# bldeng/AA-ADMM

Measured on AMD Instinct MI355X. Metric: ADMM iters/sec + time-to-eps (primal+dual residual), higher is better.
Workload: dtype f64

## Files before the change

aa-admm_amd/csrc/elastic.cpp:

```cpp
#include "elastic.hpp"

#include <algorithm>
#include <chrono>
#include <cmath>
#include <cstdio>
#include <cstdlib>
#include <cstring>
#include <memory>
#include <numeric>
#include <set>

#include "dense_gpu.hpp"
#include "spd_direct.hpp"

namespace aa {

ElasticSolver::~ElasticSolver() {
    drop_graph();
    if (ev_fork_) (void)hipEventDestroy(ev_fork_);
    if (ev_join_) (void)hipEventDestroy(ev_join_);
    if (side_) (void)hipStreamDestroy(side_);
    for (auto& kv : kstats_)
        for (auto e : kv.second.ev) (void)hipEventDestroy(e);
}
// ... 440 lines not shown
            double v = 0;
            while (k2 < r.size() && r[k2].first == r[k].first) v += r[k2++].second;
            out.push_back({r[k].first, v});
            k = k2;
        }
        rows[q] = std::move(out);
    }
    CsrMatrix A;
    A.n = nf_;
    A.ptr.assign(nf_ + 1, 0);
    for (int q = 0; q < nf_; ++q) A.ptr[q + 1] = A.ptr[q] + (int)rows[q].size();
    A.col.resize(A.ptr[nf_]);
    A.val.resize(A.ptr[nf_]);
#pragma omp parallel for schedule(static)
    for (int q = 0; q < nf_; ++q)
        for (size_t k = 0; k < rows[q].size(); ++k) { A.col[A.ptr[q] + k] = rows[q][k].first; A.val[A.ptr[q] + k] = rows[q][k].second; }
    std::vector<std::vector<std::pair<int, double>>>().swap(rows);
    stamp("assembly of A_s");
    SupernodalFactor F;
    try {
        auto pf = make_part_factor(P > 1 ? comm_ : nullptr, rank_, s());
        F = factor_on_device(A, tree, s(), pf.get());
    } catch (const Error&) {
        throw;
    } catch (const std::runtime_error& e) {
        throw Error(ERR_NUMERIC, e.what());
    }
    pipe_z_ = st_.variant == AA_VARIANT_Z && st_.acceleration_type == 1;
    if (const char* e = std::getenv("AA_Z_PIPELINE")) pipe_z_ = pipe_z_ && e[0] != '0';
    conc_ = pipe_z_ && !comm_;
    if (const char* e = std::getenv("AA_CONCURRENT")) conc_ = conc_ && e[0] != '0';
    win_u_ = conc_;
    if (const char* e = std::getenv("AA_Z_WINDOW")) win_u_ = win_u_ && e[0] != '0';
    stamp("factor");
    solver_.default_branches = (P == 1 && st_.variant == AA_VARIANT_Z) ? 2 : 1;
    solver_.build(F, s(), P > 1 ? &tree.part : nullptr, rank_, top_beg_, comm_, pipe_z_ ? 2 : 1,
                  st_.variant == AA_VARIANT_Z && st_.acceleration_type == 1);
    stamp("solver build + upload");

    std::vector<HostGroup> owned;
    nbg_ = 0;
    long long zmax = 0;
    if (P > 1) {
        std::vector<int> qpart(n, -1);
        for (int r = 0; r < P; ++r) for (int q = tree.part_beg[r]; q < tree.part_end[r]; ++q) qpart[q] = r;
        std::vector<long long> zr(P, 0);
        std::vector<int> br(P, 0);
        long long rr = 0;
        for (auto& hg : hgroups_) {
            const int cnt = (int)(hg.idx.size() / hg.nv);
            std::vector<int> c(P, 0);
            HostGroup lg;
            lg.kind = hg.kind; lg.material = hg.material; lg.nv = hg.nv; lg.ncol = hg.ncol; lg.lame = hg.lame;
            for (int t = 0; t < cnt; ++t) {
                int o = -1;
                for (int a = 0; a < hg.nv && o < 0; ++a) o = qpart[node2int_[hg.idx[(size_t)t * hg.nv + a]]];
                if (o < 0) o = (int)(rr++ % P);
                ++c[o];
                if (o != rank_) continue;
                lg.append_element(hg, (size_t)t);
            }
            for (int r = 0; r < P; ++r) { br[r] += blocks_for(c[r]); zr[r] += 3LL * hg.ncol * c[r]; }
            owned.push_back(std::move(lg));
        }
        for (int r = 0; r < P; ++r) { nbg_ = std::max(nbg_, br[r]); zmax = std::max(zmax, zr[r]); }
    }
// ... 222 lines not shown
    if (!pins_dirty_) return;
    std::vector<double> p(3 * (size_t)np_);
    int q = 0;
    for (auto& kv : pins_) { for (int j = 0; j < 3; ++j) p[3 * q + j] = kv.second[j]; ++q; }
    if (np_) {
        const size_t off = 3 * (size_t)nf_;
        AA_HIP(hipMemcpyAsync(xfull_.p + off, p.data(), p.size() * 8, hipMemcpyHostToDevice, s()));
        AA_HIP(hipMemcpyAsync(xlast_.p + off, p.data(), p.size() * 8, hipMemcpyHostToDevice, s()));
        AA_HIP(hipMemcpyAsync(cxfull_.p + off, p.data(), p.size() * 8, hipMemcpyHostToDevice, s()));
        AA_HIP(hipStreamSynchronize(s()));
    }
    pins_dirty_ = false;
}

void ElasticSolver::ev_begin(const char* name) {
    if (!instrument_) return;
    hipEvent_t e;
    AA_HIP(hipEventCreate(&e));
    AA_HIP(hipEventRecord(e, s()));
    kstats_[name].ev.push_back(e);
}
void ElasticSolver::ev_end(const char* name) { ev_begin(name); }

void ElasticSolver::local_z_all(const double* xfull, const double* u, double* z, double* y, int mode, bool red) {
    int off = 0;
    const bool timed = mode == LZ_NORMAL && red;
    if (timed) ev_begin("local_z");
    for (auto& g : groups_) {
        launch_local_z(g.d, xfull, u, z, y, nf_, st_.variant, mode, ctrl_.p, red ? pa_ : nullptr, off, s(),
                       use_queue_ ? &lq_ : nullptr, g.var, mesh_table(g.d));
        off += blocks_for(g.d.count);
    }
    if (timed) ev_end("local_z");
}

void ElasticSolver::local_z_on(const double* xfull, const double* u, double* z, int mode, hipStream_t st, Ctrl* c,
                               const LocalQueue* q) {
    for (auto& g : groups_)
        launch_local_z(g.d, xfull, u, z, nullptr, nf_, st_.variant, mode, c, nullptr, 0, st, use_queue_ ? q : nullptr,
                       g.var, mesh_table(g.d));
}

void ElasticSolver::prologue() {
    upload_pins();
    const bool accel = st_.acceleration_type == 1;
    Ctrl c;
    std::memset(&c, 0, sizeof(c));
    c.prev_prim = 1e20;
    c.cap = hist_cap_;
    c.aa_m = accel ? st_.anderson_m : 0;
    c.aa_active = accel ? 1 : 0;
    c.hist_clock = hist_clock_.p;
    c.eps_rel = st_.eps_rel;
    AA_HIP(hipMemcpyAsync(ctrl_.p, &c, sizeof(Ctrl), hipMemcpyHostToDevice, s()));
    launch_stamp(ctrl_.p, s());
    for (auto& w : winds_)
        launch_wind(w->dtris.p, w->dord.p, w->dlvl.p, w->nlvl, xs_.p, vs_.p, w->dir[0], w->dir[1], w->dir[2],
                    st_.timestep_s, s());
    launch_predict(n_, nf_, xs_.p, vs_.p, mass_.p, st_.timestep_s, st_.gravity, xbar_.p, Mxbar_.p, xfull_.p, s());
    if (comm_ && rank_ != 0 && top_beg_ < nf_)
        AA_HIP(hipMemsetAsync(Mxbar_.p + 3 * (size_t)top_beg_, 0, 3 * sizeof(double) * (size_t)(nf_ - top_beg_), s()));
    for (auto& g : groups_) launch_init_z(g.d, xfull_.p, z_.p, s());
    double* u0 = u_at(-1);
    if (Z_) AA_HIP(hipMemsetAsync(u0, 0, sizeof(double) * (size_t)Z_, s()));
    const long long nx = 3LL * nf_;
    if (st_.variant == AA_VARIANT_UX) {
        local_z_all(xfull_.p, u_.p, z_.p, y_.p, LZ_INIT, false);
        launch_rhs(nf_, dt_ptr_.p, nullptr, nullptr, y_.p, Mxbar_.p, pdt2_, b_.p, nullptr, 0, s());
        solver_.solve(b_.p, xfull_.p, nullptr, 0, s());
        {
            int off = 0;
            for (auto& g : groups_) {
                launch_resid_update_u(g.d, xfull_.p, xlast_.p, z_.p, u_.p, nf_, ctrl_.p, pa_, pb_, off, s());
// ... 24 lines not shown
    reduce_partials();
    launch_check_restore_ux(c, ga_, nbg_, accel, u_.p, xfull_.p, accel ? aa_cur_.p : nullptr, du_.p, dx_.p,
                            Z_, nx, s());
    if (accel) {
        local_z_all(xfull_.p, u_.p, z_.p, y_.p, LZ_REDO, true);
        reduce_partials();
    }
    ev_begin("rhs");
    launch_rhs(nf_, dt_ptr_.p, nullptr, nullptr, y_.p, Mxbar_.p, pdt2_, b_.p, c, 0, s(), xfull_.p, xlast_.p,
               ga_, nbg_);
    ev_end("rhs");
    ev_begin("solve");
    solver_.solve(b_.p, xfull_.p, c, 0, s());
    ev_end("solve");
    ev_begin("resid");
    {
        int off = 0;
        for (auto& g : groups_) {
            launch_resid_update_u(g.d, xfull_.p, xlast_.p, z_.p, u_.p, nf_, c, pa_, pb_, off, s());
            off += blocks_for(g.d.count);
        }
    }
    ev_end("resid");
    reduce_partials();
    if (accel) {
        const int m = st_.anderson_m;
        Seg2 G{u_.p, Z_, xfull_.p, nx};
        Seg2 cp{du_.p, Z_, dx_.p, nx};
        ev_begin("aa");
        launch_aa_reduce(G, aa_cur_.p, Z_, aa_dF_.p, aa_dG_.p, c, aa_red_.p, aa_blocks_, cp, m, s(), ga_, gb_, nbg_,
                         hist_prim_.p, hist_comb_.p, hist_rej_.p);
        reduce_aa();
        launch_aa_solve(c, aag_, aa_blocks_, m, s());
        launch_aa_mix(G, aa_cur_.p, Z_, aa_dF_.p, aa_dG_.p, c, G, m, s());
        ev_end("aa");
    } else {
        launch_control(CTL_COMB_UX, c, ga_, gb_, nbg_, accel, hist_prim_.p, hist_comb_.p, hist_rej_.p, s());
    }
}

void ElasticSolver::enqueue_iteration_z(bool accel, int it) {
    const long long nx = 3LL * nf_;
    Ctrl* c = ctrl_.p;
    const bool pipe = accel && pipe_z_;
    double *duc = du_at(it), *dzc = dz_at(it), *dxc = dx_at(it);
    double *dup = du_at(it - 1), *dzp = dz_at(it - 1), *dxp = dx_at(it - 1);
    const bool side = pipe && it > 0 && conc_;
    auto side_pass = [&](hipStream_t st) {
        comb_finish_z(CTL_COMB_ZP, st, ctrl_c_.p, red_c_.p, red_c_.p + nbg_, &lq2_, dup, dzp);
    };
    double* u = u_at(it);
    const double* ui = win_u_ ? dup : u_.p;
    ev_begin("grad");
    for (auto& g : groups_) launch_u_and_y(g.d, xfull_.p, z_.p, u, u, y_.p, nf_, accel ? 1 : 0, 0, c, s(), g.var);
    ev_end("grad");
    ev_begin("rhs");
    launch_rhs(nf_, dt_ptr_.p, nullptr, nullptr, y_.p, Mxbar_.p, pdt2_, b_.p, c, 0, s());
    ev_end("rhs");
    if (pipe && it > 0) {
        ev_begin("solve");
        solver_.solve2(b_.p, xfull_.p, b2_.p, cxfull_.p, c, 0, s());
        ev_end("solve");
        if (side) {
            launch_ctrl_fork(c, ctrl_c_.p, s());
        } else {
            ev_begin("comb");
            comb_finish_z(CTL_COMB_ZP, s(), c, pa_, pb_, &lq_, dup, dzp);
// ... 30 lines not shown
    if (accel) {
        const int m = st_.anderson_m;
        auto copy_defaults = [&]() {
            ev_begin("copy");
            launch_copy(dxc, xfull_.p, nx, c, 0, s());
            if (!win_u_) launch_copy(duc, u_.p, Z_, c, 0, s());
            ev_end("copy");
        };
        if (instrument_) copy_defaults();
        ev_begin("local_z");
        local_z_all(xfull_.p, u, dzc, y_.p, LZ_NORMAL, false);
        ev_end("local_z");
        if (side && instrument_) {
            ev_begin("comb");
            side_pass(s());
            ev_end("comb");
            join_wait_ = false;
        }
        Seg2 G{dzc, Z_, nullptr, 0};
        Seg2 out{z_.p, Z_, nullptr, 0};
        Seg2 none{nullptr, 0, nullptr, 0};
        ev_begin("aa");
        launch_aa_reduce(G, z_.p, Z_, aa_dF_.p, aa_dG_.p, c, aa_red_.p, aa_blocks_, none, m, s());
        reduce_aa();
        if (side && !instrument_) {
            AA_HIP(hipEventRecord(ev_fork_, s()));
            AA_HIP(hipStreamWaitEvent(side_, ev_fork_, 0));
            side_pass(side_);
            AA_HIP(hipEventRecord(ev_join_, side_));
            join_wait_ = true;
        }
        if (!instrument_) copy_defaults();
        launch_aa_solve(c, aag_, aa_blocks_, m, s());
        launch_aa_mix(G, z_.p, Z_, aa_dF_.p, aa_dG_.p, c, out, m, s());
        ev_end("aa");
        if (pipe) {
            ev_begin("rhs");
            launch_rhs(nf_, dt_ptr_.p, nullptr, nullptr, y_.p, Mxbar_.p, pdt2_, b2_.p, c, 0, s());
            ev_end("rhs");
            if (side) {
                join_dx_ = dxp;
                join_side();
            }
            return;
        }
        ev_begin("comb");
        launch_rhs(nf_, dt_ptr_.p, nullptr, nullptr, y_.p, Mxbar_.p, pdt2_, b_.p, c, 0, s());
        solver_.solve(b_.p, cxfull_.p, c, 0, s());
        comb_finish_z(CTL_COMB_Z, s(), c, pa_, pb_, &lq_, duc, dzc);
        ev_end("comb");
        return;
    }
    launch_copy(lastz_.p, z_.p, Z_, c, 0, s());
    ev_begin("local_z");
    local_z_all(xfull_.p, u, z_.p, nullptr, LZ_NORMAL, false);
    ev_end("local_z");
    prim_all(xfull_.p, z_.p, lastz_.p, 0);
    reduce_partials();
    launch_control(CTL_COMB_Z, c, ga_, gb_, nbg_, accel, hist_prim_.p, hist_comb_.p, hist_rej_.p, s());
}

void ElasticSolver::comb_finish_z(int op, hipStream_t st, Ctrl* c, double* pa, double* pb, const LocalQueue* q,
                                  const double* du, const double* dz) {
    local_z_on(cxfull_.p, du, cz_.p, LZ_NORMAL, st, c, q);
    int off = 0;
    for (auto& g : groups_) {
        launch_prim_z(g.d, cxfull_.p, cz_.p, dz, nf_, 0, c, pa, pb, off, st);
        off += blocks_for(g.d.count);
    }
    if (st == s()) {
        reduce_partials();
        launch_control(op, c, ga_, gb_, nbg_, 1, hist_prim_.p, hist_comb_.p, hist_rej_.p, st);
    } else {
        launch_control(op, c, pa, pb, nbg_, 1, hist_prim_.p, hist_comb_.p, hist_rej_.p, st);
    }
}

void ElasticSolver::join_side() {
    if (join_wait_) AA_HIP(hipStreamWaitEvent(s(), ev_join_, 0));
    launch_ctrl_join(ctrl_.p, ctrl_c_.p, xfull_.p, join_dx_, 3LL * nf_, s());
}

void ElasticSolver::enqueue_comb_tail_z(int iters) {
    ev_begin("comb");
    solver_.solve(b2_.p, cxfull_.p, ctrl_.p, 0, s());
    comb_finish_z(CTL_COMB_Z, s(), ctrl_.p, pa_, pb_, &lq_, du_at(iters - 1), dz_at(iters - 1));
    ev_end("comb");
}

void ElasticSolver::enqueue_iterations(int iters, bool accel) {
    static const int eager_sync = [] { const char* e = std::getenv("AA_EAGER_SYNC"); return e ? std::atoi(e) : 0; }();
    hipStreamCaptureStatus cst = hipStreamCaptureStatusNone;
    if (eager_sync > 0) AA_HIP(hipStreamIsCapturing(s(), &cst));
    for (int it = 0; it < iters; ++it) {
        if (st_.variant == AA_VARIANT_UX) enqueue_iteration_ux(accel);
        else enqueue_iteration_z(accel, it);
        if (eager_sync > 0 && cst == hipStreamCaptureStatusNone && (it + 1) % eager_sync == 0)
            AA_HIP(hipStreamSynchronize(s()));
    }
    if (st_.variant != AA_VARIANT_UX && accel && pipe_z_ && iters > 0) enqueue_comb_tail_z(iters);
// ... 179 lines not shown
```

aa-admm_amd/csrc/elastic.hpp:

```cpp
#pragma once
#include <array>
#include <map>
#include <memory>
#include <string>
#include <vector>

#include "../../include/aa_admm.h"
#include "comm.hpp"
#include "common.hpp"
#include "direct_solve.hpp"
#include "elastic_kernels.hpp"
#include "mesh_obstacle.hpp"

namespace aa {

struct Context {
    int device = 0;
    hipStream_t stream = nullptr;
};

struct MeshObsBuffers {
    DevBuf<BvhNode> nodes;
    DevBuf<BvhTri> tris;
    DevBuf<double> pn;
// ... 120 lines not shown
    int red_blocks_ = 0, aa_blocks_ = 0, hist_cap_ = 0;
    Comm* comm_ = nullptr;
    int rank_ = 0, own_beg_ = 0, own_end_ = 0, top_beg_ = 0;
    void reduce_partials();
    void reduce_aa();
    void gather_state(DevBuf<double>& v);
    std::vector<double> h_prim_, h_comb_;
    std::vector<int> h_rej_;
    int nrec_ = 0;
    aa_runtime rt_{};
    std::vector<std::pair<std::string, double>> setup_phases_;
    bool pins_dirty_ = true;

    hipGraph_t graph_ = nullptr;
    hipGraphExec_t gexec_ = nullptr;
    bool use_graph_ = true;
    bool pipe_z_ = false;
    void drop_graph();
    bool conc_ = false;
    bool join_wait_ = false;
    double* join_dx_ = nullptr;
    void join_side();
    hipStream_t side_ = nullptr;
    hipEvent_t ev_fork_ = nullptr, ev_join_ = nullptr;
    DevBuf<Ctrl> ctrl_c_;
    DevBuf<int> lzq2_;
    LocalQueue lq2_;
    DevBuf<double> red_c_, du2_, dz2_, dx2_;
    double* du_at(int it) { return conc_ && (it & 1) ? du2_.p : du_.p; }
    double* dz_at(int it) { return conc_ && (it & 1) ? dz2_.p : dz_.p; }
    double* dx_at(int it) { return conc_ && (it & 1) ? dx2_.p : dx_.p; }
    bool win_u_ = false;
    double* u_at(int it) { return win_u_ ? du_at(it) : u_.p; }

    bool instrument_ = false;
    struct KStat { std::vector<hipEvent_t> ev; double bytes = 0; double total_ms = 0; int launches = 0; };
    std::map<std::string, KStat> kstats_;
    void ev_begin(const char* name);
    void ev_end(const char* name);

    void upload_pins();
    void prologue();
    void enqueue_iteration_ux(bool accel);
    void enqueue_iteration_z(bool accel, int it);
    void comb_finish_z(int op, hipStream_t st, Ctrl* c, double* pa, double* pb, const LocalQueue* q,
                       const double* du, const double* dz);
    void enqueue_comb_tail_z(int iters);
    void enqueue_iterations(int iters, bool accel);
    void epilogue_enqueue(bool accel);
    void fetch_results();
    int nb_elems() const { return red_blocks_; }
    void local_z_all(const double* xfull, const double* u, double* z, double* y, int mode, bool red);
    void local_z_on(const double* xfull, const double* u, double* z, int mode, hipStream_t st, Ctrl* c,
                    const LocalQueue* q);
};

}
```

aa-admm_amd/csrc/elastic_kernels.hip:

```cpp
#include <algorithm>
#include <cstdlib>

#include "common.hpp"
#include "device_lbfgs.hpp"
#include "device_prox.hpp"
#include "elastic_kernels.hpp"

namespace aa {

namespace {

__device__ __forceinline__ double wave_sum(double v) {
#pragma unroll
    for (int o = 32; o > 0; o >>= 1) v += __shfl_down(v, o, 64);
    return v;
}

__device__ __forceinline__ double block_sum(double v, double* sm) {
    v = wave_sum(v);
    const int lane = threadIdx.x & 63, wid = threadIdx.x >> 6;
    if (lane == 0) sm[wid] = v;
    __syncthreads();
    double r = 0;
    if (threadIdx.x == 0)
// ... 124 lines not shown
    double gk[NC * NV];
#pragma unroll
    for (int a = 0; a < NV; ++a) pos[a] = g.spos[(size_t)a * g.count + e];
#pragma unroll
    for (int k = 0; k < NC * NV; ++k) gk[k] = g.G[(size_t)k * g.count + e];
#pragma unroll
    for (int a = 0; a < NV; ++a) {
        if (pos[a] < 0) continue;
        double f0 = 0, f1 = 0, f2 = 0;
#pragma unroll
        for (int c = 0; c < NC; ++c) {
            const double gc = gk[c * NV + a];
            f0 += gc * yc[3 * c]; f1 += gc * yc[3 * c + 1]; f2 += gc * yc[3 * c + 2];
        }
        double* o = y + 3 * (size_t)pos[a];
        o[0] = f0; o[1] = f1; o[2] = f2;
    }
}

template <int D>
__device__ __forceinline__ void load_u(const GroupDev& g, int e, const double* __restrict__ u, double* uu) {
    if (u) {
#pragma unroll
        for (int i = 0; i < D; ++i) uu[i] = u[g.zoff + (size_t)i * g.count + e];
    } else {
#pragma unroll
        for (int i = 0; i < D; ++i) uu[i] = 0.0;
    }
}

template <class... V>
constexpr bool kVar = sizeof...(V) != 0;
__device__ __forceinline__ const GroupVar& var_of(const GroupVar& v) { return v; }
template <bool VAR>
struct LaneMat {};
template <>
struct LaneMat<true> {
    double mu = 0, lambda = 0, k = 0;
};

template <int NV, int HYPER, class... V>
__global__ __launch_bounds__(kBlock) void k_local_z(GroupDev g, const double* __restrict__ xfull,
                                                    const double* __restrict__ u, double* __restrict__ z,
                                                    double* __restrict__ y, int nf, int variant, int mode, Ctrl* ctrl,
                                                    double* red, int red_off, V... gvp) {
    constexpr bool VAR = kVar<V...>;
    if (mode != LZ_INIT && gated(ctrl, mode == LZ_REDO)) return;
    __shared__ double sm[kBlock / 64];
    constexpr int NC = ncol_of(NV), D = 3 * NC;
    const int e = blockIdx.x * blockDim.x + threadIdx.x;
    double part = 0;
    if (e < g.count) {
        double F[D], Cp[D], uu[D], vin[D], zz[D];
        gather_F<NV>(g, e, xfull, nf, F, Cp);
        const double w = g.w[e];
        load_u<D>(g, e, u, uu);
#pragma unroll
        for (int i = 0; i < D; ++i) vin[i] = F[i] + uu[i] / w;
        if constexpr (NV == 1) {
            if (variant == 1) dev::collision_candidate(F, uu, w, vin);
            if constexpr (VAR) dev::collision_prox(vin, g.obs, zz, gvp...);
            else dev::collision_prox(vin, g.obs, zz);
        } else if constexpr (NV == 3) {
            if constexpr (VAR) dev::tri_prox(vin, zz, variant, var_of(gvp...).lmin[e], var_of(gvp...).lmax[e]);
            else dev::tri_prox(vin, zz, variant, g.lmin, g.lmax);
        } else if constexpr (HYPER == 0) {
// ... 122 lines not shown
                    }
                }
            }
        }
        bool fin = false;
        if constexpr (VAR) fin = active && L.iterate(g.mat, M.mu, M.lambda, M.k, vol, v, x, &fail);
        else fin = active && L.iterate(g.mat, g.mu, g.lambda, g.k, vol, v, x, &fail);
        if (fin) {
            active = false;
            pending = true;
            if (stats) atomicAdd(&hist[min(L.k_it, 100)], 1u);
        }
    }
    if (stats) {
        if (lane == 0) {
            atomicAdd(stats + 101, (unsigned long long)trips);
            atomicAdd(stats + 102, (unsigned long long)refills);
            atomicAdd(stats + 103, 1ull);
        }
        __syncthreads();
        for (int i = threadIdx.x; i < 101; i += blockDim.x)
            if (hist[i]) atomicAdd(stats + i, (unsigned long long)hist[i]);
    }
    if (fail && ctrl) ctrl->fail = 1;
    queue_reset_last(queue);
}

template <int NV, bool SLOTS = true, class... V>
__global__ __launch_bounds__(kBlock) void k_local_z_hqf(GroupDev g, const double* __restrict__ xfull,
                                                        const double* __restrict__ u, double* __restrict__ z,
                                                        double* __restrict__ y, int nf, int mode, Ctrl* ctrl,
                                                        int* __restrict__ queue, int refill,
                                                        unsigned long long* __restrict__ stats, V... gvp) {
    constexpr bool VAR = kVar<V...>;
    static_assert(NV == 4, "the fused refill is for tets");
    if (mode != LZ_INIT && gated(ctrl, mode == LZ_REDO)) return;
    unsigned trips = 0, refills = 0;
    __shared__ unsigned hist[101];
    if (stats) {
        for (int i = threadIdx.x; i < 101; i += blockDim.x) hist[i] = 0;
        __syncthreads();
    }
    constexpr int NC = ncol_of(NV), D = 3 * NC;
    const int lane = threadIdx.x & 63;
    dev::HyperLbfgs L;
    [[maybe_unused]] LaneMat<VAR> M;
    double v[D], x[D];
    double vol = 0;
    int e = 0, fail = 0;
    bool active = false, pending = false, exhausted = false;
    const size_t n = g.count;
    for (;;) {
        const bool need = !active && !exhausted;
        const unsigned long long mask = __ballot(need);
        if (!__any(active || need)) break;
        ++trips;
        if (mask && (__popcll(mask) >= refill || !__any(active))) {
            ++refills;
            const int leader = __ffsll((long long)mask) - 1;
            const int rank = __popcll(mask & ((1ull << lane) - 1ull));
            int b = 0;
            if (lane == leader) b = queue_claim(queue, __popcll(mask));
            int so[NV];
            double go[NC * NV], uo[D], wo = 1.0;
            if (SLOTS && y) {
#pragma unroll
                for (int a = 0; a < NV; ++a) so[a] = g.spos[a * n + e];
#pragma unroll
                for (int k = 0; k < NC * NV; ++k) go[k] = g.G[k * n + e];
                load_u<D>(g, e, u, uo);
                wo = g.w[e];
            }
            b = __shfl(b, leader, 64);
            const int my = b + rank;
            const int en = min(my, g.count - 1);
            int id[NV];
#pragma unroll
            for (int a = 0; a < NV; ++a) id[a] = g.idx[a * n + en];
            if (pending) {
#pragma unroll
                for (int i = 0; i < D; ++i) z[g.zoff + (size_t)i * n + e] = x[i];
                if (SLOTS && y) {
                    double Cp[D];
#pragma unroll
                    for (int i = 0; i < D; ++i) Cp[i] = 0;
                    write_slots_pre<NV>(so, go, wo, x, Cp, uo, y);
                }
                pending = false;
            }
            double xp[3 * NV], gn[NC * NV], un[D];
#pragma unroll
            for (int a = 0; a < NV; ++a) {
                xp[3 * a] = xfull[3 * (size_t)id[a]];
                xp[3 * a + 1] = xfull[3 * (size_t)id[a] + 1];
                xp[3 * a + 2] = xfull[3 * (size_t)id[a] + 2];
            }
#pragma unroll
            for (int k = 0; k < NC * NV; ++k) gn[k] = g.G[k * n + en];
            load_u<D>(g, en, u, un);
            const double wn = g.w[en], voln = g.vol[en];
            [[maybe_unused]] double mun = 0, lamn = 0, kn = 0;
            if constexpr (VAR) {
                const GroupVar& gv = var_of(gvp...);
                mun = gv.mu[en]; lamn = gv.lambda[en]; kn = gv.k[en];
            }
            if (need) {
                if (my >= g.count) {
                    exhausted = true;
                } else {
                    e = my;
                    double F[D];
#pragma unroll
                    for (int i = 0; i < D; ++i) F[i] = 0;
#pragma unroll
                    for (int a = 0; a < NV; ++a)
#pragma unroll
                        for (int c = 0; c < NC; ++c) {
                            const double gc = gn[c * NV + a];
                            F[3 * c + 0] += gc * xp[3 * a]; F[3 * c + 1] += gc * xp[3 * a + 1];
                            F[3 * c + 2] += gc * xp[3 * a + 2];
                        }
#pragma unroll
                    for (int i = 0; i < D; ++i) {
                        v[i] = F[i] + un[i] / wn;
                        x[i] = v[i];
                    }
                    vol = voln;
                    bool ok;
                    if constexpr (VAR) {
                        M.mu = mun; M.lambda = lamn; M.k = kn;
                        ok = L.start(g.mat, M.mu, M.lambda, M.k, vol, v, x);
                    } else {
                        ok = L.start(g.mat, g.mu, g.lambda, g.k, vol, v, x);
                    }
                    if (ok) {
                        pending = true;
                        if (stats) atomicAdd(&hist[0], 1u);
                    } else {
                        active = true;
                    }
                }
            }
        }
        bool fin = false;
        if constexpr (VAR) fin = active && L.iterate(g.mat, M.mu, M.lambda, M.k, vol, v, x, &fail);
        else fin = active && L.iterate(g.mat, g.mu, g.lambda, g.k, vol, v, x, &fail);
        if (fin) {
            active = false;
            pending = true;
            if (stats) atomicAdd(&hist[min(L.k_it, 100)], 1u);
        }
    }
    if (stats) {
        if (lane == 0) {
            atomicAdd(stats + 101, (unsigned long long)trips);
            atomicAdd(stats + 102, (unsigned long long)refills);
            atomicAdd(stats + 103, 1ull);
        }
// ... 231 lines not shown
}

template <int NV>
__global__ __launch_bounds__(kBlock) void k_prim_z(GroupDev g, const double* __restrict__ xfull,
                                                   const double* __restrict__ z, const double* __restrict__ zref,
                                                   int nf, int redo, Ctrl* ctrl, double* red_a, double* red_b,
                                                   int red_off) {
    if (gated(ctrl, redo)) return;
    __shared__ double sm[kBlock / 64];
    constexpr int NC = ncol_of(NV), D = 3 * NC;
    const int e = blockIdx.x * blockDim.x + threadIdx.x;
    double pa = 0, pb = 0;
    if (e < g.count) {
        double F[D];
        gather_P<NV>(g, e, xfull, F);
        const double w = g.w[e];
        double zi[D], zr[D];
#pragma unroll
        for (int i = 0; i < D; ++i) zi[i] = z[g.zoff + (size_t)i * g.count + e];
        if (zref) {
#pragma unroll
            for (int i = 0; i < D; ++i) zr[i] = zref[g.zoff + (size_t)i * g.count + e];
        }
#pragma unroll
        for (int i = 0; i < D; ++i) {
            const double r = w * (F[i] - zi[i]);
            pa += r * r;
            if (zref) { const double d = w * (zi[i] - zr[i]); pb += d * d; }
        }
    }
    const double sa = block_sum(pa, sm);
    const double sb = block_sum(pb, sm);
    if (threadIdx.x == 0) { red_a[red_off + blockIdx.x] = sa; if (red_b) red_b[red_off + blockIdx.x] = sb; }
}

template <int NV>
__global__ __launch_bounds__(kBlock) void k_init_z(GroupDev g, const double* __restrict__ xfull, double* __restrict__ z) {
    constexpr int NC = ncol_of(NV), D = 3 * NC;
    const int e = blockIdx.x * blockDim.x + threadIdx.x;
    if (e >= g.count) return;
    double F[D];
    gather_P<NV>(g, e, xfull, F);
#pragma unroll
    for (int i = 0; i < D; ++i) z[g.zoff + (size_t)i * g.count + e] = F[i];
}

__global__ __launch_bounds__(kBlock) void k_rhs(int nf, const int* __restrict__ ptr, const int* __restrict__ row,
                                                const double* __restrict__ val, const double* __restrict__ y,
                                                const double* __restrict__ Mxbar, double pdt2, double* __restrict__ b,
                                                Ctrl* ctrl, int gate_reject, const double* __restrict__ xsrc,
                                                double* __restrict__ xlast, const double* __restrict__ red_final,
                                                int nb_final) {
    if (gated(ctrl, gate_reject)) return;
    if (red_final && blockIdx.x == 0) {
        __shared__ double sm[kBlock / 64];
        const double a = block_sum_all(red_final, nb_final, sm);
        if (threadIdx.x == 0) {
            if (ctrl->reject) ctrl->prim = sqrt(a);
            ctrl->prev_prim = ctrl->prim;
        }
    }
    const int i = blockIdx.x * blockDim.x + threadIdx.x;
    if (i >= nf) return;
    if (xlast) {
        xlast[3 * (size_t)i] = xsrc[3 * (size_t)i];
        xlast[3 * (size_t)i + 1] = xsrc[3 * (size_t)i + 1];
// ... 825 lines not shown
        } else if (var) {
            const int rf = queue->refill_lanes;
            if (!queue->fused || g.pinned)
                hipLaunchKernelGGL((k_local_z_hq<4, GroupVar>), grid, dim3(kBlock), 0, s, g, xfull, u, z, y, nf, mode, ctrl,
                                   queue->counter, rf, queue->stats, var);
            else if (y)
                hipLaunchKernelGGL((k_local_z_hqf<4, true, GroupVar>), grid, dim3(kBlock), 0, s, g, xfull, u, z, y, nf, mode,
                                   ctrl, queue->counter, rf, queue->stats, var);
            else
                hipLaunchKernelGGL((k_local_z_hqf<4, false, GroupVar>), grid, dim3(kBlock), 0, s, g, xfull, u, z, y, nf,
                                   mode, ctrl, queue->counter, rf, queue->stats, var);
        } else if (!queue->fused || g.pinned)
            hipLaunchKernelGGL((k_local_z_hq<4>), grid, dim3(kBlock), 0, s, g, xfull, u, z, y, nf, mode, ctrl,
                               queue->counter, refill, queue->stats);
        else if (y)
            hipLaunchKernelGGL((k_local_z_hqf<4, true>), grid, dim3(kBlock), 0, s, g, xfull, u, z, y, nf, mode,
                               ctrl, queue->counter, refill, queue->stats);
        else
            hipLaunchKernelGGL((k_local_z_hqf<4, false>), grid, dim3(kBlock), 0, s, g, xfull, u, z, y, nf, mode,
                               ctrl, queue->counter, refill, queue->stats);
        AA_CHECK_LAUNCH();
        return;
    }
    if (g.kind == 2 && meshes) hipLaunchKernelGGL((k_local_z<1, 0, const MeshObsDev*>), dim3(nb), dim3(kBlock), 0, s, g, xfull, u, z, y, nf, variant, mode, ctrl, red, red_off, meshes);
    else if (g.kind == 2) hipLaunchKernelGGL((k_local_z<1, 0>), dim3(nb), dim3(kBlock), 0, s, g, xfull, u, z, y, nf, variant, mode, ctrl, red, red_off);
    else if (g.kind == 1 && var) hipLaunchKernelGGL((k_local_z<3, 0, GroupVar>), dim3(nb), dim3(kBlock), 0, s, g, xfull, u, z, y, nf, variant, mode, ctrl, red, red_off, var);
    else if (g.kind == 1) hipLaunchKernelGGL((k_local_z<3, 0>), dim3(nb), dim3(kBlock), 0, s, g, xfull, u, z, y, nf, variant, mode, ctrl, red, red_off);
    else if (g.mat == 0) hipLaunchKernelGGL((k_local_z<4, 0>), dim3(nb), dim3(kBlock), 0, s, g, xfull, u, z, y, nf, variant, mode, ctrl, red, red_off);
    else if (var) hipLaunchKernelGGL((k_local_z<4, 1, GroupVar>), dim3(nb), dim3(kBlock), 0, s, g, xfull, u, z, y, nf, variant, mode, ctrl, red, red_off, var);
    else hipLaunchKernelGGL((k_local_z<4, 1>), dim3(nb), dim3(kBlock), 0, s, g, xfull, u, z, y, nf, variant, mode, ctrl, red, red_off);
    AA_CHECK_LAUNCH();
}

void launch_resid_update_u(const GroupDev& g, const double* xfull, const double* xlast, const double* z, double* u,
                           int nf, Ctrl* ctrl, double* red_a, double* red_b, int red_off, hipStream_t s) {
    if (g.count == 0) return;
    const int nb = blocks_for(g.count);
    if (g.kind == 2) hipLaunchKernelGGL(k_resid_u<1>, dim3(nb), dim3(kBlock), 0, s, g, xfull, xlast, z, u, nf, ctrl, red_a, red_b, red_off);
    else if (g.kind == 1) hipLaunchKernelGGL(k_resid_u<3>, dim3(nb), dim3(kBlock), 0, s, g, xfull, xlast, z, u, nf, ctrl, red_a, red_b, red_off);
    else hipLaunchKernelGGL(k_resid_u<4>, dim3(nb), dim3(kBlock), 0, s, g, xfull, xlast, z, u, nf, ctrl, red_a, red_b, red_off);
    AA_CHECK_LAUNCH();
}

void launch_u_and_y(const GroupDev& g, const double* xfull, const double* z, const double* uin, double* u, double* y,
                    int nf, int mode, int redo, Ctrl* ctrl, hipStream_t s, const GroupVar& var) {
    if (g.count == 0) return;
    const int nb = blocks_for(g.count);
    if (g.kind == 2) hipLaunchKernelGGL((k_u_and_y<1, 0>), dim3(nb), dim3(kBlock), 0, s, g, xfull, z, uin, u, y, nf, mode, redo, ctrl);
    else if (g.kind == 1) hipLaunchKernelGGL((k_u_and_y<3, 0>), dim3(nb), dim3(kBlock), 0, s, g, xfull, z, uin, u, y, nf, mode, redo, ctrl);
    else if (g.mat == 0 && var) hipLaunchKernelGGL((k_u_and_y<4, 0, GroupVar>), dim3(nb), dim3(kBlock), 0, s, g, xfull, z, uin, u, y, nf, mode, redo, ctrl, var);
    else if (g.mat == 0) hipLaunchKernelGGL((k_u_and_y<4, 0>), dim3(nb), dim3(kBlock), 0, s, g, xfull, z, uin, u, y, nf, mode, redo, ctrl);
    else if (var) hipLaunchKernelGGL((k_u_and_y<4, 1, GroupVar>), dim3(nb), dim3(kBlock), 0, s, g, xfull, z, uin, u, y, nf, mode, redo, ctrl, var);
    else hipLaunchKernelGGL((k_u_and_y<4, 1>), dim3(nb), dim3(kBlock), 0, s, g, xfull, z, uin, u, y, nf, mode, redo, ctrl);
    AA_CHECK_LAUNCH();
}

void launch_prim_z(const GroupDev& g, const double* xfull, const double* z, const double* zref, int nf, int redo,
                   Ctrl* ctrl, double* red_a, double* red_b, int red_off, hipStream_t s) {
    if (g.count == 0) return;
    const int nb = blocks_for(g.count);
    if (g.kind == 2) hipLaunchKernelGGL(k_prim_z<1>, dim3(nb), dim3(kBlock), 0, s, g, xfull, z, zref, nf, redo, ctrl, red_a, red_b, red_off);
    else if (g.kind == 1) hipLaunchKernelGGL(k_prim_z<3>, dim3(nb), dim3(kBlock), 0, s, g, xfull, z, zref, nf, redo, ctrl, red_a, red_b, red_off);
    else hipLaunchKernelGGL(k_prim_z<4>, dim3(nb), dim3(kBlock), 0, s, g, xfull, z, zref, nf, redo, ctrl, red_a, red_b, red_off);
    AA_CHECK_LAUNCH();
}

// ... 163 lines not shown
static bool aa_cols() {
    static const bool on = !(std::getenv("AA_AA_COLS") && std::getenv("AA_AA_COLS")[0] == '0');
    return on;
}

void launch_aa_reduce(Seg2 G, const double* cur, long long eff, double* dF, double* dG, Ctrl* ctrl, double* red,
                      int nblocks, Seg2 copy_to, int m, hipStream_t s, const double* comb_a, const double* comb_b,
                      int comb_nb, double* hist_prim, double* hist_comb, int* hist_rej, AAMask mask) {
#define AA_RED_ARGS G, cur, eff, dF, dG, ctrl, red, copy_to, comb_a, comb_b, comb_nb, hist_prim, hist_comb, hist_rej, mask
    switch (mm_bucket(m)) {
        case 8: hipLaunchKernelGGL(k_aa_reduce<8>, dim3(nblocks), dim3(kBlock), 0, s, AA_RED_ARGS); break;
        case 12: hipLaunchKernelGGL(k_aa_reduce<12>, dim3(nblocks), dim3(kBlock), 0, s, AA_RED_ARGS); break;
        case 16: hipLaunchKernelGGL(k_aa_reduce<16>, dim3(nblocks), dim3(kBlock), 0, s, AA_RED_ARGS); break;
        default:
            if (aa_cols()) hipLaunchKernelGGL(k_aa_reduce_cols<32>, dim3(nblocks), dim3(kBlock), 0, s, AA_RED_ARGS);
            else hipLaunchKernelGGL(k_aa_reduce<32>, dim3(nblocks), dim3(kBlock), 0, s, AA_RED_ARGS);
            break;
    }
#undef AA_RED_ARGS
    AA_CHECK_LAUNCH();
}

void launch_aa_solve(Ctrl* ctrl, const double* red, int nblocks, int m, hipStream_t s) {
    switch (mm_bucket(m)) {
        case 8: hipLaunchKernelGGL(k_aa_solve<8>, dim3(1), dim3(kSolveBlock), 0, s, ctrl, red, nblocks); break;
        case 12: hipLaunchKernelGGL(k_aa_solve<12>, dim3(1), dim3(kSolveBlock), 0, s, ctrl, red, nblocks); break;
        case 16: hipLaunchKernelGGL(k_aa_solve<16>, dim3(1), dim3(kSolveBlock), 0, s, ctrl, red, nblocks); break;
        default: hipLaunchKernelGGL(k_aa_solve<32>, dim3(1), dim3(kSolveBlock), 0, s, ctrl, red, nblocks); break;
    }
    AA_CHECK_LAUNCH();
}

void launch_aa_mix(Seg2 G, double* cur, long long eff, double* dF, double* dG, Ctrl* ctrl, Seg2 out, int m,
                   hipStream_t s) {
    const long long dim = G.na + G.nb;
    switch (mm_bucket(m)) {
        case 8: hipLaunchKernelGGL(k_aa_mix<8>, dim3(grid_for(dim)), dim3(kBlock), 0, s, G, cur, eff, dF, dG, ctrl, out); break;
        case 12: hipLaunchKernelGGL(k_aa_mix<12>, dim3(grid_for(dim)), dim3(kBlock), 0, s, G, cur, eff, dF, dG, ctrl, out); break;
        case 16: hipLaunchKernelGGL(k_aa_mix<16>, dim3(grid_for(dim)), dim3(kBlock), 0, s, G, cur, eff, dF, dG, ctrl, out); break;
        default: hipLaunchKernelGGL(k_aa_mix<32>, dim3(grid_for(dim)), dim3(kBlock), 0, s, G, cur, eff, dF, dG, ctrl, out); break;
    }
    AA_CHECK_LAUNCH();
}

void launch_test_prox(int op, const double* prm4, const double* in, int n, double* out, int* iters, hipStream_t s) {
    if (n <= 0) return;
    hipLaunchKernelGGL(k_test_prox, dim3((n + 63) / 64), dim3(64), 0, s, op, prm4[0], prm4[1], prm4[2], prm4[3], in, n, out,
                       iters);
    AA_CHECK_LAUNCH();
}

void launch_test_cod(int n, const double* M, const double* b, double* x, hipStream_t s) {
    hipLaunchKernelGGL(k_test_cod, dim3(1), dim3(kSolveBlock), 0, s, n, M, b, x);
    AA_CHECK_LAUNCH();
}

void launch_test_mesh_sdf(const MeshObsDev* mesh, const double* q, int n, double* closest, double* dx, int* tri,
                          hipStream_t s) {
    if (n <= 0) return;
    hipLaunchKernelGGL(k_test_mesh_sdf, dim3(blocks_for(n)), dim3(kBlock), 0, s, mesh, q, n, closest, dx, tri);
    AA_CHECK_LAUNCH();
}

void launch_test_collision_prox(const double* obs, const MeshObsDev* meshes, const double* q, int n, double* out,
                                hipStream_t s) {
    if (n <= 0) return;
    hipLaunchKernelGGL(k_test_collision_prox, dim3(blocks_for(n)), dim3(kBlock), 0, s, obs, meshes, q, n, out);
    AA_CHECK_LAUNCH();
}
// ... 40 lines not shown
```

aa-admm_amd/csrc/elastic_kernels.hpp:

```cpp
#pragma once
#include <hip/hip_runtime.h>

#include "bvh.hpp"

namespace aa {

constexpr int kMaxM = 32;
constexpr double kCombEps = 1e-20;

struct GroupDev {
    int kind;
    int mat;
    int count;
    int nv, ncol, dim;
    int pinned;
    long long zoff;
    long long yrow;
    const int* idx;
    const int* spos;
    const double* G;
    const double* w;
    const double* vol;
    double mu, lambda, k, lmin, lmax;
    const double* obs;
// ... 24 lines not shown
    long long clock0;
    double eps_rel, eps_abs;
    int eps_hit, pad_;
};
void launch_stamp(Ctrl* ctrl, hipStream_t s);

struct Seg2 {
    double* a; long long na;
    double* b; long long nb;
};

struct AAMask {
    long long lo1 = 0, hi1 = 0x7fffffffffffffffLL, lo2 = 0, hi2 = 0;
};

struct ElasticLaunch;

enum LocalMode { LZ_NORMAL = 0, LZ_REDO = 1, LZ_INIT = 2 };

struct LocalQueue {
    int* counter = nullptr;
    int resident = 0, refill = 60;
    int refill_lanes = 60;
    bool fused = false;
    bool split = false;
    unsigned long long* stats = nullptr;
};
constexpr int kLqStats = 104;
LocalQueue make_local_queue(int device, int* counter);
void launch_local_z(const GroupDev& g, const double* xfull, const double* u, double* z, double* y, int nf,
                    int variant, int mode, Ctrl* ctrl, double* red, int red_off, hipStream_t s,
                    const LocalQueue* queue = nullptr, const GroupVar& var = GroupVar(),
                    const MeshObsDev* meshes = nullptr);
void launch_resid_update_u(const GroupDev& g, const double* xfull, const double* xlast, const double* z, double* u,
                           int nf, Ctrl* ctrl, double* red_a, double* red_b, int red_off, hipStream_t s);
void launch_u_and_y(const GroupDev& g, const double* xfull, const double* z, const double* uin, double* u, double* y,
                    int nf, int mode, int redo, Ctrl* ctrl, hipStream_t s, const GroupVar& var = GroupVar());
void launch_prim_z(const GroupDev& g, const double* xfull, const double* z, const double* zref, int nf, int redo,
                   Ctrl* ctrl, double* red_a, double* red_b, int red_off, hipStream_t s);
void launch_rhs(int nf, const int* ptr, const int* row, const double* val, const double* y, const double* Mxbar,
                double pdt2, double* b, Ctrl* ctrl, int gate_reject, hipStream_t s,
                const double* xsrc = nullptr, double* xlast = nullptr, const double* red_final = nullptr,
                int nb_final = 0);
void launch_check_restore_z(Ctrl* ctrl, const double* red, int nb, int accel, double* u, double* x, double* z,
                            const double* du, const double* dx, const double* dz, long long nz, long long nx,
                            hipStream_t s);
void launch_check_restore_ux(Ctrl* ctrl, const double* red, int nb, int accel, double* u, double* x, double* cur,
                             const double* du, const double* dx, long long nz, long long nx, hipStream_t s);
void launch_restore_ux(double* u, double* x, double* cur, const double* du, const double* dx, long long nz,
                       long long nx, const Ctrl* ctrl, hipStream_t s);
enum CtlOp { CTL_PRIM_CHECK = 0, CTL_PRIM_FINAL = 1, CTL_COMB_UX = 2, CTL_PRIM_CHECK_Z = 3, CTL_PRIM_FINAL_Z = 4,
             CTL_COMB_Z = 5, CTL_COMB_ZP = 6 };
void launch_control(int op, Ctrl* ctrl, const double* red_a, const double* red_b, int nblocks, int accel,
                    double* hist_prim, double* hist_comb, int* hist_rej, hipStream_t s);
void launch_ctrl_fork(const Ctrl* ctrl, Ctrl* side, hipStream_t s);
void launch_ctrl_join(Ctrl* ctrl, const Ctrl* side, double* x, const double* dx, long long n, hipStream_t s);
void launch_copy(double* dst, const double* src, long long n, const Ctrl* ctrl, int gate_reject, hipStream_t s);
double bench_stream_read(long long bytes, int reps, hipStream_t s);
void launch_predict(int n, int nf, double* xstate, double* vstate, const double* mass, double dt, double gravity,
                    double* xbar, double* Mxbar, double* xfull, hipStream_t s);
void launch_init_z(const GroupDev& g, const double* xfull, double* z, hipStream_t s);
void launch_finalize(int n, int nf, const double* xsrc, const double* xfull, double* xstate, double* vstate, double dt,
                     hipStream_t s);
void launch_wind(const int* tris3, const int* tri_ord, const int* lvl_ptr, int nlvl, const double* x, double* v,
                 double dir0, double dir1, double dir2, double dt, hipStream_t s);

int aa_window_bucket(int m);
int aa_reduce_blocks(long long dim);
void launch_aa_reduce(Seg2 G, const double* cur, long long eff, double* dF, double* dG, Ctrl* ctrl, double* red,
                      int nblocks, Seg2 copy_to, int m, hipStream_t s, const double* comb_a = nullptr,
                      const double* comb_b = nullptr, int comb_nb = 0, double* hist_prim = nullptr,
                      double* hist_comb = nullptr, int* hist_rej = nullptr, AAMask mask = AAMask());
void launch_aa_solve(Ctrl* ctrl, const double* red, int nblocks, int m, hipStream_t s);
void launch_aa_mix(Seg2 G, double* cur, long long eff, double* dF, double* dG, Ctrl* ctrl, Seg2 out, int m,
                   hipStream_t s);

void launch_test_prox(int op, const double* prm4, const double* in, int n, double* out, int* iters, hipStream_t s);
void launch_test_cod(int n, const double* M, const double* b, double* x, hipStream_t s);
void launch_test_mesh_sdf(const MeshObsDev* mesh, const double* q, int n, double* closest, double* dx, int* tri,
                          hipStream_t s);
void launch_test_collision_prox(const double* obs, const MeshObsDev* meshes, const double* q, int n, double* out,
                                hipStream_t s);

}
```

Before: 456.0.

## Fuse combined-residual computation into local z kernel and narrow AA mix templates

In the combined-step finish for the Z variant, the local z solve now computes each element's primal and dual residual contributions directly and writes two per-element scalars instead of the full z vector. A light k_prim_sum kernel then reduces those scalars, replacing the prim_z kernel that re-read xfull, z and dz. Separately, the AA mix kernel gets exact template instances for m≤6 and m=7 so it does not run with the wider m=8 bucket. This cuts memory traffic and per-thread work, but cz_ now holds residual scalars rather than z values, and the local kernel carries extra per-lane registers.

```diff
diff --git a/aa-admm_amd/csrc/elastic.cpp b/aa-admm_amd/csrc/elastic.cpp
--- a/aa-admm_amd/csrc/elastic.cpp
+++ b/aa-admm_amd/csrc/elastic.cpp
@@ -496,6 +496,8 @@
     if (const char* e = std::getenv("AA_CONCURRENT")) conc_ = conc_ && e[0] != '0';
     win_u_ = conc_;
     if (const char* e = std::getenv("AA_Z_WINDOW")) win_u_ = win_u_ && e[0] != '0';
+    comb_fused_ = true;
+    if (const char* e = std::getenv("AA_COMB_FUSED")) comb_fused_ = e[0] != '0';
     stamp("factor");
     solver_.default_branches = (P == 1 && st_.variant == AA_VARIANT_Z) ? 2 : 1;
     solver_.build(F, s(), P > 1 ? &tree.part : nullptr, rank_, top_beg_, comm_, pipe_z_ ? 2 : 1,
@@ -784,13 +786,6 @@
         off += blocks_for(g.d.count);
     }
     if (timed) ev_end("local_z");
-}
-
-void ElasticSolver::local_z_on(const double* xfull, const double* u, double* z, int mode, hipStream_t st, Ctrl* c,
-                               const LocalQueue* q) {
-    for (auto& g : groups_)
-        launch_local_z(g.d, xfull, u, z, nullptr, nf_, st_.variant, mode, c, nullptr, 0, st, use_queue_ ? q : nullptr,
-                       g.var, mesh_table(g.d));
 }
 
 void ElasticSolver::prologue() {
@@ -881,7 +876,7 @@
                          hist_prim_.p, hist_comb_.p, hist_rej_.p);
         reduce_aa();
         launch_aa_solve(c, aag_, aa_blocks_, m, s());
-        launch_aa_mix(G, aa_cur_.p, Z_, aa_dF_.p, aa_dG_.p, c, G, m, s());
+        launch_aa_mix(G, aa_cur_.p, Z_, aa_dF_.p, aa_dG_.p, c, G, m, s(), comb_fused_);
         ev_end("aa");
     } else {
         launch_control(CTL_COMB_UX, c, ga_, gb_, nbg_, accel, hist_prim_.p, hist_comb_.p, hist_rej_.p, s());
@@ -978,7 +973,7 @@
         }
         if (!instrument_) copy_defaults();
         launch_aa_solve(c, aag_, aa_blocks_, m, s());
-        launch_aa_mix(G, z_.p, Z_, aa_dF_.p, aa_dG_.p, c, out, m, s());
+        launch_aa_mix(G, z_.p, Z_, aa_dF_.p, aa_dG_.p, c, out, m, s(), comb_fused_);
         ev_end("aa");
         if (pipe) {
             ev_begin("rhs");
@@ -1008,10 +1003,17 @@
 
 void ElasticSolver::comb_finish_z(int op, hipStream_t st, Ctrl* c, double* pa, double* pb, const LocalQueue* q,
                                   const double* du, const double* dz) {
-    local_z_on(cxfull_.p, du, cz_.p, LZ_NORMAL, st, c, q);
+    const LocalQueue* lq = use_queue_ ? q : nullptr;
+    auto fused = [&](const DevGroup& g) { return comb_fused_ && local_z_res_ok(g.d, lq); };
+    for (auto& g : groups_) {
+        if (fused(g)) launch_local_z_res(g.d, cxfull_.p, du, dz, cz_.p, nf_, c, st, lq, g.var);
+        else launch_local_z(g.d, cxfull_.p, du, cz_.p, nullptr, nf_, st_.variant, LZ_NORMAL, c, nullptr, 0, st, lq, g.var,
+                            mesh_table(g.d));
+    }
     int off = 0;
     for (auto& g : groups_) {
-        launch_prim_z(g.d, cxfull_.p, cz_.p, dz, nf_, 0, c, pa, pb, off, st);
+        if (fused(g)) launch_prim_sum(g.d, cz_.p, c, pa, pb, off, st);
+        else launch_prim_z(g.d, cxfull_.p, cz_.p, dz, nf_, 0, c, pa, pb, off, st);
         off += blocks_for(g.d.count);
     }
     if (st == s()) {
diff --git a/aa-admm_amd/csrc/elastic.hpp b/aa-admm_amd/csrc/elastic.hpp
--- a/aa-admm_amd/csrc/elastic.hpp
+++ b/aa-admm_amd/csrc/elastic.hpp
@@ -176,6 +176,7 @@
     double* dx_at(int it) { return conc_ && (it & 1) ? dx2_.p : dx_.p; }
     bool win_u_ = false;
     double* u_at(int it) { return win_u_ ? du_at(it) : u_.p; }
+    bool comb_fused_ = true;
 
     bool instrument_ = false;
     struct KStat { std::vector<hipEvent_t> ev; double bytes = 0; double total_ms = 0; int launches = 0; };
@@ -195,8 +196,6 @@
     void fetch_results();
     int nb_elems() const { return red_blocks_; }
     void local_z_all(const double* xfull, const double* u, double* z, double* y, int mode, bool red);
-    void local_z_on(const double* xfull, const double* u, double* z, int mode, hipStream_t st, Ctrl* c,
-                    const LocalQueue* q);
 };
 
 }
diff --git a/aa-admm_amd/csrc/elastic_kernels.hip b/aa-admm_amd/csrc/elastic_kernels.hip
--- a/aa-admm_amd/csrc/elastic_kernels.hip
+++ b/aa-admm_amd/csrc/elastic_kernels.hip
@@ -180,6 +180,16 @@
 template <class... V>
 constexpr bool kVar = sizeof...(V) != 0;
 __device__ __forceinline__ const GroupVar& var_of(const GroupVar& v) { return v; }
+struct ResArgs {
+    const double* zref;
+};
+template <class... V>
+constexpr bool kRes = false;
+template <class... V>
+constexpr bool kRes<ResArgs, V...> = true;
+__device__ __forceinline__ const GroupVar& var_of(const ResArgs&, const GroupVar& v) { return v; }
+__device__ __forceinline__ const ResArgs& res_of(const ResArgs& r) { return r; }
+__device__ __forceinline__ const ResArgs& res_of(const ResArgs& r, const GroupVar&) { return r; }
 template <bool VAR>
 struct LaneMat {};
 template <>
@@ -368,8 +378,9 @@
                                                         double* __restrict__ y, int nf, int mode, Ctrl* ctrl,
                                                         int* __restrict__ queue, int refill,
                                                         unsigned long long* __restrict__ stats, V... gvp) {
-    constexpr bool VAR = kVar<V...>;
+    constexpr bool RES = kRes<V...>, VAR = sizeof...(V) > (RES ? 1 : 0);
     static_assert(NV == 4, "the fused refill is for tets");
+    static_assert(!(RES && SLOTS), "the residual form writes no slots");
     if (mode != LZ_INIT && gated(ctrl, mode == LZ_REDO)) return;
     unsigned trips = 0, refills = 0;
     __shared__ unsigned hist[101];
@@ -382,6 +393,7 @@
     dev::HyperLbfgs L;
     [[maybe_unused]] LaneMat<VAR> M;
     double v[D], x[D];
+    [[maybe_unused]] double Fk[RES ? D : 1];
     double vol = 0;
     int e = 0, fail = 0;
     bool active = false, pending = false, exhausted = false;
@@ -407,6 +419,12 @@
                 load_u<D>(g, e, u, uo);
                 wo = g.w[e];
             }
+            [[maybe_unused]] double zr[RES ? D : 1];
+            if constexpr (RES) {
+#pragma unroll
+                for (int i = 0; i < D; ++i) zr[i] = res_of(gvp...).zref[g.zoff + (size_t)i * n + e];
+                wo = g.w[e];
+            }
             b = __shfl(b, leader, 64);
             const int my = b + rank;
             const int en = min(my, g.count - 1);
@@ -414,8 +432,21 @@
 #pragma unroll
             for (int a = 0; a < NV; ++a) id[a] = g.idx[a * n + en];
             if (pending) {
-#pragma unroll
-                for (int i = 0; i < D; ++i) z[g.zoff + (size_t)i * n + e] = x[i];
+                if constexpr (RES) {
+                    double pa = 0, pb = 0;
+#pragma unroll
+                    for (int i = 0; i < D; ++i) {
+                        const double r = wo * (Fk[i] - x[i]);
+                        pa += r * r;
+                        const double d = wo * (x[i] - zr[i]);
+                        pb += d * d;
+                    }
+                    z[g.zoff + e] = pa;
+                    z[g.zoff + n + e] = pb;
+                } else {
+#pragma unroll
+                    for (int i = 0; i < D; ++i) z[g.zoff + (size_t)i * n + e] = x[i];
+                }
                 if (SLOTS && y) {
                     double Cp[D];
 #pragma unroll
@@ -460,6 +491,7 @@
                     for (int i = 0; i < D; ++i) {
                         v[i] = F[i] + un[i] / wn;
                         x[i] = v[i];
+                        if constexpr (RES) Fk[i] = F[i];
                     }
                     vol = voln;
                     bool ok;
@@ -757,6 +789,21 @@
     const double sa = block_sum(pa, sm);
     const double sb = block_sum(pb, sm);
     if (threadIdx.x == 0) { red_a[red_off + blockIdx.x] = sa; if (red_b) red_b[red_off + blockIdx.x] = sb; }
+}
+
+__global__ __launch_bounds__(kBlock) void k_prim_sum(GroupDev g, const double* __restrict__ pe, Ctrl* ctrl,
+                                                     double* red_a, double* red_b, int red_off) {
+    if (gated(ctrl, 0)) return;
+    __shared__ double sm[kBlock / 64];
+    const int e = blockIdx.x * blockDim.x + threadIdx.x;
+    double pa = 0, pb = 0;
+    if (e < g.count) {
+        pa = pe[g.zoff + e];
+        pb = pe[g.zoff + (size_t)g.count + e];
+    }
+    const double sa = block_sum(pa, sm);
+    const double sb = block_sum(pb, sm);
+    if (threadIdx.x == 0) { red_a[red_off + blockIdx.x] = sa; red_b[red_off + blockIdx.x] = sb; }
 }
 
 template <int NV>
@@ -1648,6 +1695,30 @@
     AA_CHECK_LAUNCH();
 }
 
+bool local_z_res_ok(const GroupDev& g, const LocalQueue* queue) {
+    return g.kind == 0 && g.mat != 0 && !g.pinned && queue && queue->counter && queue->fused && !queue->split;
+}
+
+void launch_local_z_res(const GroupDev& g, const double* xfull, const double* u, const double* zref, double* pe, int nf,
+                        Ctrl* ctrl, hipStream_t s, const LocalQueue* queue, const GroupVar& var) {
+    if (g.count == 0) return;
+    const dim3 grid(std::min(blocks_for(g.count), std::max(1, queue->resident)));
+    if (var)
+        hipLaunchKernelGGL((k_local_z_hqf<4, false, ResArgs, GroupVar>), grid, dim3(kBlock), 0, s, g, xfull, u, pe, nullptr,
+                           nf, (int)LZ_NORMAL, ctrl, queue->counter, queue->refill_lanes, queue->stats, ResArgs{zref}, var);
+    else
+        hipLaunchKernelGGL((k_local_z_hqf<4, false, ResArgs>), grid, dim3(kBlock), 0, s, g, xfull, u, pe, nullptr, nf,
+                           (int)LZ_NORMAL, ctrl, queue->counter, queue->refill, queue->stats, ResArgs{zref});
+    AA_CHECK_LAUNCH();
+}
+
+void launch_prim_sum(const GroupDev& g, const double* pe, Ctrl* ctrl, double* red_a, double* red_b, int red_off,
+                     hipStream_t s) {
+    if (g.count == 0) return;
+    hipLaunchKernelGGL(k_prim_sum, dim3(blocks_for(g.count)), dim3(kBlock), 0, s, g, pe, ctrl, red_a, red_b, red_off);
+    AA_CHECK_LAUNCH();
+}
+
 void launch_resid_update_u(const GroupDev& g, const double* xfull, const double* xlast, const double* z, double* u,
                            int nf, Ctrl* ctrl, double* red_a, double* red_b, int red_off, hipStream_t s) {
     if (g.count == 0) return;
@@ -1877,9 +1948,11 @@
 }
 
 void launch_aa_mix(Seg2 G, double* cur, long long eff, double* dF, double* dG, Ctrl* ctrl, Seg2 out, int m,
-                   hipStream_t s) {
+                   hipStream_t s, bool narrow) {
     const long long dim = G.na + G.nb;
-    switch (mm_bucket(m)) {
+    switch (narrow && m <= 6 ? 6 : (narrow && m == 7 ? 7 : mm_bucket(m))) {
+        case 6: hipLaunchKernelGGL(k_aa_mix<6>, dim3(grid_for(dim)), dim3(kBlock), 0, s, G, cur, eff, dF, dG, ctrl, out); break;
+        case 7: hipLaunchKernelGGL(k_aa_mix<7>, dim3(grid_for(dim)), dim3(kBlock), 0, s, G, cur, eff, dF, dG, ctrl, out); break;
         case 8: hipLaunchKernelGGL(k_aa_mix<8>, dim3(grid_for(dim)), dim3(kBlock), 0, s, G, cur, eff, dF, dG, ctrl, out); break;
         case 12: hipLaunchKernelGGL(k_aa_mix<12>, dim3(grid_for(dim)), dim3(kBlock), 0, s, G, cur, eff, dF, dG, ctrl, out); break;
         case 16: hipLaunchKernelGGL(k_aa_mix<16>, dim3(grid_for(dim)), dim3(kBlock), 0, s, G, cur, eff, dF, dG, ctrl, out); break;
diff --git a/aa-admm_amd/csrc/elastic_kernels.hpp b/aa-admm_amd/csrc/elastic_kernels.hpp
--- a/aa-admm_amd/csrc/elastic_kernels.hpp
+++ b/aa-admm_amd/csrc/elastic_kernels.hpp
@@ -80,6 +80,11 @@
                     int variant, int mode, Ctrl* ctrl, double* red, int red_off, hipStream_t s,
                     const LocalQueue* queue = nullptr, const GroupVar& var = GroupVar(),
                     const MeshObsDev* meshes = nullptr);
+bool local_z_res_ok(const GroupDev& g, const LocalQueue* queue);
+void launch_local_z_res(const GroupDev& g, const double* xfull, const double* u, const double* zref, double* pe, int nf,
+                        Ctrl* ctrl, hipStream_t s, const LocalQueue* queue, const GroupVar& var = GroupVar());
+void launch_prim_sum(const GroupDev& g, const double* pe, Ctrl* ctrl, double* red_a, double* red_b, int red_off,
+                     hipStream_t s);
 void launch_resid_update_u(const GroupDev& g, const double* xfull, const double* xlast, const double* z, double* u,
                            int nf, Ctrl* ctrl, double* red_a, double* red_b, int red_off, hipStream_t s);
 void launch_u_and_y(const GroupDev& g, const double* xfull, const double* z, const double* uin, double* u, double* y,
@@ -121,7 +126,7 @@
                       double* hist_comb = nullptr, int* hist_rej = nullptr, AAMask mask = AAMask());
 void launch_aa_solve(Ctrl* ctrl, const double* red, int nblocks, int m, hipStream_t s);
 void launch_aa_mix(Seg2 G, double* cur, long long eff, double* dF, double* dG, Ctrl* ctrl, Seg2 out, int m,
-                   hipStream_t s);
+                   hipStream_t s, bool narrow = true);
 
 void launch_test_prox(int op, const double* prm4, const double* in, int n, double* out, int* iters, hipStream_t s);
 void launch_test_cod(int n, const double* M, const double* b, double* x, hipStream_t s);
```

New measurement: 471.0, median of 6. 3.3% higher.
